# gkv856/speaker_embedding_GE2E_loss

Measured on NVIDIA B200. Metric: GE2E fwd+bwd utterances/s, higher is better.
Workload: dtype tf32

## Files before the change

### speaker_embedding_ge2e_loss_b200/csrc/ge2e_simt.cu

```cuda
#include <cuda_fp16.h>
#include <limits.h>

#include <algorithm>
#include <stdlib.h>

#include <initializer_list>

#include "ge2e_common.cuh"
#include "ge2e_tc_ptx.cuh"

namespace ge2e {

namespace {

constexpr int kThreads = 256;
constexpr int kWarps = kThreads / kWarp;
constexpr int kStreamRows = 32;

enum { MODE_FWD = 0, MODE_BWD_DE = 1, MODE_BWD_DC = 2 };

__device__ __forceinline__ float4 ld4(const float* __restrict__ row, int col, int D, bool vec) {
  float4 v = make_float4(0.f, 0.f, 0.f, 0.f);
  if (vec) {
    if (col < D) v = __ldg(reinterpret_cast<const float4*>(row + col));
// ... 67 lines not shown
  }
  __syncthreads();

  const float m1 = (float)(M - 1);
  for (int i = wid; i < M; i += kWarps) {
    float ne2 = 0.f, nu2 = 0.f, eu = 0.f;
    for (int d = lane << 2; d < Dp; d += 128) {
      const float4 e = *reinterpret_cast<const float4*>(&sE[(size_t)i * Dp + d]);
      const float4 s = *reinterpret_cast<const float4*>(&sS[d]);
      float4 u;
      u.x = (s.x - e.x) / m1; u.y = (s.y - e.y) / m1; u.z = (s.z - e.z) / m1; u.w = (s.w - e.w) / m1;
      ne2 += dot4(e, e);
      nu2 += dot4(u, u);
      eu += dot4(e, u);
    }
    ne2 = warp_sum(ne2); nu2 = warp_sum(nu2); eu = warp_sum(eu);
    const float inv_ne = 1.f / fmaxf(sqrtf(ne2), kCosDelta);
    const float inv_nu = 1.f / fmaxf(sqrtf(nu2), kCosDelta);
    float* out = e_hat + ((size_t)j * M + i) * D;
    for (int d = lane << 2; d < Dp; d += 128) {
      float4 e = *reinterpret_cast<const float4*>(&sE[(size_t)i * Dp + d]);
      e.x *= inv_ne; e.y *= inv_ne; e.z *= inv_ne; e.w *= inv_ne;
      if (ROUND) { e.x = round_tf32(e.x); e.y = round_tf32(e.y); e.z = round_tf32(e.z); e.w = round_tf32(e.w); }
      st4(out, d, D, vec_out, e);
    }
    if (lane == 0) cos_diag[(size_t)j * M + i] = eu * inv_ne * inv_nu;
  }

  float part = 0.f;
  const float fm = (float)M;
  for (int d = tid; d < Dp; d += kThreads) {
    const float c = sS[d] / fm;
    part += c * c;
  }
  const float tot = block_sum(part, red);
  if (tid == 0) s_inv_nc = 1.f / fmaxf(sqrtf(tot), kCosDelta);
  __syncthreads();
  const float inv_nc = s_inv_nc;
  for (int d = tid; d < D; d += kThreads) {
    float c = (sS[d] / fm) * inv_nc;
    if (ROUND) c = round_tf32(c);
    c_hat[(size_t)j * D + d] = c;
  }
}

template <bool ROUND>
__global__ void __launch_bounds__(kThreads)
prep_kernel(const float* __restrict__ E, const int32_t* __restrict__ idx, int M, int D, int Dp,
            float* __restrict__ e_hat, float* __restrict__ c_hat, float* __restrict__ cos_diag,
            float* __restrict__ accum) {
  extern __shared__ __align__(16) float smem[];
  if (blockIdx.x == 0 && threadIdx.x < 4 && accum != nullptr) accum[threadIdx.x] = 0.f;
  prep_body<ROUND>(E, idx, blockIdx.x, M, D, Dp, e_hat, c_hat, cos_diag, smem);
}


template <int PREC>
__device__ __forceinline__ void put4(float* base, size_t row, int D, int col, float4 v) {
  if (PREC == 3) {
    __half* h = reinterpret_cast<__half*>(base);
    const __half2 h0 = __floats2half2_rn(v.x, v.y), h1 = __floats2half2_rn(v.z, v.w);
    uint2 hi;
    hi.x = *reinterpret_cast<const uint32_t*>(&h0); hi.y = *reinterpret_cast<const uint32_t*>(&h1);
    *reinterpret_cast<uint2*>(h + row * 2 * D + col) = hi;
  } else if (PREC == 2) {
    __half* h = reinterpret_cast<__half*>(base);
    const __half2 h0 = __floats2half2_rn(v.x, v.y), h1 = __floats2half2_rn(v.z, v.w);
    const float2 f0 = __half22float2(h0), f1 = __half22float2(h1);
    const __half2 l0 = __floats2half2_rn(v.x - f0.x, v.y - f0.y), l1 = __floats2half2_rn(v.z - f1.x, v.w - f1.y);
    uint2 hi, lo;
    hi.x = *reinterpret_cast<const uint32_t*>(&h0); hi.y = *reinterpret_cast<const uint32_t*>(&h1);
    lo.x = *reinterpret_cast<const uint32_t*>(&l0); lo.y = *reinterpret_cast<const uint32_t*>(&l1);
    *reinterpret_cast<uint2*>(h + row * 2 * D + col) = hi;
    *reinterpret_cast<uint2*>(h + row * 2 * D + D + col) = lo;
  } else {
    if (PREC == 1) { v.x = round_tf32(v.x); v.y = round_tf32(v.y); v.z = round_tf32(v.z); v.w = round_tf32(v.w); }
    *reinterpret_cast<float4*>(base + row * D + col) = v;
  }
}

constexpr int kPrepWarps = 4;
constexpr int kRowBatch = 4;
constexpr int kRegRows = 16;

template <int KCH, int PREC>
__global__ void __launch_bounds__(kPrepWarps * 32)
prep_warp_kernel(const float* __restrict__ E, const int32_t* __restrict__ idx, int n_local, int M,
                 float* __restrict__ e_hat, float* __restrict__ c_hat, float* __restrict__ cos_diag,
                 float* __restrict__ accum) {
  constexpr int D = KCH * 128;
  const int lane = threadIdx.x & 31, wid = threadIdx.x >> 5;
  const int j = blockIdx.x * kPrepWarps + wid;
  pdl_wait();
  pdl_trigger();
  if (blockIdx.x == 0 && threadIdx.x < 4 && accum != nullptr) accum[threadIdx.x] = 0.f;
  if (j >= n_local) return;
  auto rowp = [&](int i) {
    return reinterpret_cast<const float4*>(E + phys_row(idx, (size_t)j * M + i) * D) + lane;
  };
  float4 s[KCH];
#pragma unroll
  for (int c = 0; c < KCH; ++c) s[c] = make_float4(0.f, 0.f, 0.f, 0.f);
  for (int i0 = 0; i0 < M; i0 += kRowBatch) {
    float4 v[kRowBatch][KCH];
#pragma unroll
    for (int r = 0; r < kRowBatch; ++r)
#pragma unroll
      for (int c = 0; c < KCH; ++c)
        v[r][c] = (i0 + r < M) ? __ldg(rowp(i0 + r) + c * 32) : make_float4(0.f, 0.f, 0.f, 0.f);
#pragma unroll
    for (int r = 0; r < kRowBatch; ++r)
#pragma unroll
      for (int c = 0; c < KCH; ++c) {
        s[c].x += v[r][c].x; s[c].y += v[r][c].y; s[c].z += v[r][c].z; s[c].w += v[r][c].w;
      }
  }
  const float inv_m = 1.f / (float)M, inv_m1 = 1.f / (float)(M - 1);
  float ss = 0.f;
#pragma unroll
  for (int c = 0; c < KCH; ++c) ss += dot4(s[c], s[c]);
  ss = warp_sum(ss);
  const float sc = inv_m / fmaxf(sqrtf(ss) * inv_m, kCosDelta);
#pragma unroll
  for (int c = 0; c < KCH; ++c)
    put4<PREC>(c_hat, j, D, 4 * lane + 128 * c,
               make_float4(s[c].x * sc, s[c].y * sc, s[c].z * sc, s[c].w * sc));
  float my_cos = 0.f;
  for (int i0 = 0; i0 < M; i0 += kRowBatch) {
    float4 v[kRowBatch][KCH];
    float ne2[kRowBatch], nd2[kRowBatch], ed[kRowBatch];
#pragma unroll
    for (int r = 0; r < kRowBatch; ++r)
#pragma unroll
      for (int c = 0; c < KCH; ++c)
        v[r][c] = (i0 + r < M) ? __ldg(rowp(i0 + r) + c * 32) : make_float4(0.f, 0.f, 0.f, 0.f);
#pragma unroll
    for (int r = 0; r < kRowBatch; ++r) {
      ne2[r] = 0.f; nd2[r] = 0.f; ed[r] = 0.f;
#pragma unroll
      for (int c = 0; c < KCH; ++c) {
        const float4 e = v[r][c];
        const float4 d = make_float4(s[c].x - e.x, s[c].y - e.y, s[c].z - e.z, s[c].w - e.w);
        ne2[r] += dot4(e, e); nd2[r] += dot4(d, d); ed[r] += dot4(e, d);
      }
    }
#pragma unroll
    for (int o = 16; o > 0; o >>= 1)
#pragma unroll
      for (int r = 0; r < kRowBatch; ++r) {
        ne2[r] += __shfl_xor_sync(0xffffffffu, ne2[r], o);
        nd2[r] += __shfl_xor_sync(0xffffffffu, nd2[r], o);
        ed[r] += __shfl_xor_sync(0xffffffffu, ed[r], o);
      }
#pragma unroll
    for (int r = 0; r < kRowBatch; ++r) {
      if (i0 + r < M) {
        const float inv_ne = 1.f / fmaxf(sqrtf(ne2[r]), kCosDelta);
        const float inv_nu = 1.f / fmaxf(sqrtf(nd2[r]) * inv_m1, kCosDelta);
        if (lane == ((i0 + r) & 31)) my_cos = (ed[r] * inv_m1) * inv_ne * inv_nu;
#pragma unroll
        for (int c = 0; c < KCH; ++c) {
          float4 e = v[r][c];
          e.x *= inv_ne; e.y *= inv_ne; e.z *= inv_ne; e.w *= inv_ne;
          put4<PREC>(e_hat, (size_t)j * M + i0 + r, D, 4 * lane + 128 * c, e);
        }
      }
    }
    if (((i0 + kRowBatch) & 31) == 0 || i0 + kRowBatch >= M) {
      const int base = (i0 + kRowBatch - 1) & ~31;
      if (base + lane < M) cos_diag[(size_t)j * M + base + lane] = my_cos;
    }
  }
}

__host__ __device__ constexpr int rev4(int i) {
  return ((i & 1) << 3) | ((i & 2) << 1) | ((i & 4) >> 1) | ((i & 8) >> 3);
}
__device__ __forceinline__ float reduce16_transposed(const float (&v)[16], int lane) {
  float a[8], b[4], c[2];
  const bool u1 = (lane & 1) != 0, u2 = (lane & 2) != 0, u4 = (lane & 4) != 0, u8 = (lane & 8) != 0;
#pragma unroll
  for (int q = 0; q < 8; ++q) a[q] = (u1 ? v[q + 8] : v[q]) + __shfl_xor_sync(0xffffffffu, u1 ? v[q] : v[q + 8], 1);
#pragma unroll
  for (int q = 0; q < 4; ++q) b[q] = (u2 ? a[q + 4] : a[q]) + __shfl_xor_sync(0xffffffffu, u2 ? a[q] : a[q + 4], 2);
#pragma unroll
  for (int q = 0; q < 2; ++q) c[q] = (u4 ? b[q + 2] : b[q]) + __shfl_xor_sync(0xffffffffu, u4 ? b[q] : b[q + 2], 4);
  const float e = (u8 ? c[1] : c[0]) + __shfl_xor_sync(0xffffffffu, u8 ? c[0] : c[1], 8);
  return e + __shfl_xor_sync(0xffffffffu, e, 16);
}

template <int KCH, int RR, int PREC>
__global__ void __launch_bounds__(kPrepWarps * 32)
prep_reg_kernel(const float* __restrict__ E, const int32_t* __restrict__ idx, int n_local, int M,
                float* __restrict__ e_hat, float* __restrict__ c_hat, float* __restrict__ cos_diag,
                float* __restrict__ accum) {
  constexpr int D = KCH * 128, R = RR;
  static_assert(R <= 16, "reduce16_transposed handles 16 rows");
  const int lane = threadIdx.x & 31, wid = threadIdx.x >> 5;
  const int j = blockIdx.x * kPrepWarps + wid;
  pdl_wait();
  pdl_trigger();
  if (blockIdx.x == 0 && threadIdx.x < 4 && accum != nullptr) accum[threadIdx.x] = 0.f;
  if (j >= n_local) return;
  float4 v[R][KCH];
#pragma unroll
  for (int i = 0; i < R; ++i) {
    const float4* rp = (i < M) ? reinterpret_cast<const float4*>(E + phys_row(idx, (size_t)j * M + i) * D) + lane : nullptr;
#pragma unroll
    for (int c = 0; c < KCH; ++c) v[i][c] = (i < M) ? __ldg(rp + c * 32) : make_float4(0.f, 0.f, 0.f, 0.f);
  }
  float4 s[KCH];
#pragma unroll
  for (int c = 0; c < KCH; ++c) {
    s[c] = v[0][c];
#pragma unroll
    for (int i = 1; i < R; ++i) { s[c].x += v[i][c].x; s[c].y += v[i][c].y; s[c].z += v[i][c].z; s[c].w += v[i][c].w; }
  }
  const float inv_m = 1.f / (float)M, inv_m1 = 1.f / (float)(M - 1);
  float ss = 0.f;
#pragma unroll
  for (int c = 0; c < KCH; ++c) ss += dot4(s[c], s[c]);
  ss = warp_sum(ss);
  const float sc = inv_m / fmaxf(sqrtf(ss) * inv_m, kCosDelta);
#pragma unroll
  for (int c = 0; c < KCH; ++c)
    put4<PREC>(c_hat, j, D, 4 * lane + 128 * c,
               make_float4(s[c].x * sc, s[c].y * sc, s[c].z * sc, s[c].w * sc));
  float ne2[16], nd2[16], ed[16];
#pragma unroll
  for (int i = R; i < 16; ++i) { ne2[i] = 0.f; nd2[i] = 0.f; ed[i] = 0.f; }
#pragma unroll
  for (int i = 0; i < R; ++i) {
    ne2[i] = 0.f; nd2[i] = 0.f; ed[i] = 0.f;
#pragma unroll
    for (int c = 0; c < KCH; ++c) {
      const float4 e = v[i][c];
      const float4 d = make_float4(s[c].x - e.x, s[c].y - e.y, s[c].z - e.z, s[c].w - e.w);
      ne2[i] += dot4(e, e); nd2[i] += dot4(d, d); ed[i] += dot4(e, d);
    }
  }
  const float t_ne2 = reduce16_transposed(ne2, lane), t_nd2 = reduce16_transposed(nd2, lane);
  const float t_ed = reduce16_transposed(ed, lane);
  const int my_row = rev4(lane & 15);
  const float inv_ne = 1.f / fmaxf(sqrtf(t_ne2), kCosDelta);
  const float inv_nu = 1.f / fmaxf(sqrtf(t_nd2) * inv_m1, kCosDelta);
  if (lane < 16 && my_row < M) cos_diag[(size_t)j * M + my_row] = (t_ed * inv_m1) * inv_ne * inv_nu;
#pragma unroll
  for (int i = 0; i < R; ++i) {
    if (i < M) {
      const float k = __shfl_sync(0xffffffffu, inv_ne, rev4(i));
#pragma unroll
      for (int c = 0; c < KCH; ++c) {
        float4 e = v[i][c];
        e.x *= k; e.y *= k; e.z *= k; e.w *= k;
        put4<PREC>(e_hat, (size_t)j * M + i, D, 4 * lane + 128 * c, e);
      }
    }
  }
}

struct StripParams {
  const float* own;
  const float* str;
  int n_own, n_str, D;
  int M, spk_offset;
  const float* cos_diag;
  const float* row_stat;
  const float* row_aux;
  float* row_aux_out;
  const float* w;
  const float* b;
  const float* grad_out;
  float eps;
  float* row_stat_out;
  int32_t* kstar_out;
  float* loss_accum;
  float* per_row_out;
  float* sim_out;
  float* acc_out;
  float* dwdb;
  int chunks_per_split;
};

template <int K, int R, int KCH>
struct RedT {
  static __device__ __forceinline__ void run(const float4 (&a)[R][KCH], const float* __restrict__ stage,
                                             int t, int lane, float (&out)[R]) {
    float lo[R], hi[R];
    RedT<K + 1, R, KCH>::run(a, stage, t, lane, lo);
    RedT<K + 1, R, KCH>::run(a, stage, t + (1 << K), lane, hi);
    const bool up = (lane & (1 << K)) != 0;
#pragma unroll
    for (int q = 0; q < R; ++q) {
      const float send = up ? lo[q] : hi[q];
      const float keep = up ? hi[q] : lo[q];
      out[q] = keep + __shfl_xor_sync(0xffffffffu, send, 1 << K);
    }
  }
};
template <int R, int KCH>
struct RedT<5, R, KCH> {
  static __device__ __forceinline__ void run(const float4 (&a)[R][KCH], const float* __restrict__ stage,
                                             int t, int lane, float (&out)[R]) {
#pragma unroll
    for (int q = 0; q < R; ++q) out[q] = 0.f;
#pragma unroll
    for (int c = 0; c < KCH; ++c) {
      const float4 bv = *reinterpret_cast<const float4*>(&stage[(size_t)t * (KCH * 128) + c * 128 + (lane << 2)]);
#pragma unroll
      for (int q = 0; q < R; ++q) out[q] += dot4(a[q][c], bv);
    }
  }
};

template <int MODE, int VARIANT, int KCH, int R>
__global__ void __launch_bounds__(kThreads)
strip_kernel(const StripParams p) {
  extern __shared__ __align__(16) float stage[];
  __shared__ float red[kWarps];
  constexpr int ROWLEN = KCH * 128;
  const int tid = threadIdx.x, lane = tid & 31, wid = tid >> 5;
  const int own0 = (blockIdx.x * kWarps + wid) * R;
  const int D = p.D;
  const bool vec_own = is_vec(p.own, D), vec_str = is_vec(p.str, D);
  const float w = __ldg(p.w), b = __ldg(p.b), eps = p.eps;
  const float g = (MODE == MODE_FWD) ? 1.f : __ldg(p.grad_out);

  float4 a[R][KCH];
#pragma unroll
  for (int q = 0; q < R; ++q) {
    const int row = own0 + q;
#pragma unroll
    for (int c = 0; c < KCH; ++c) {
      const int col = (lane << 2) + c * 128;
      a[q][c] = (row < p.n_own) ? ld4(p.own + (size_t)row * D, col, D, vec_own) : make_float4(0.f, 0.f, 0.f, 0.f);
    }
  }

  int jg[R];
// ... 420 lines not shown
    float ne2[kRowBatch], nd2[kRowBatch], ed[kRowBatch], eg[kRowBatch];
#pragma unroll
    for (int r = 0; r < kRowBatch; ++r) {
      ne2[r] = 0.f; nd2[r] = 0.f; ed[r] = 0.f; eg[r] = 0.f;
#pragma unroll
      for (int c = 0; c < KCH; ++c) {
        const bool in = i0 + r < M;
        v[r][c] = in ? __ldg(rowp(i0 + r) + c * 32) : make_float4(0.f, 0.f, 0.f, 0.f);
        const float4 gv = in ? __ldg(Gj + (size_t)(i0 + r) * (D / 4) + c * 32) : make_float4(0.f, 0.f, 0.f, 0.f);
        const float4 e = v[r][c];
        const float4 d = make_float4(s[c].x - e.x, s[c].y - e.y, s[c].z - e.z, s[c].w - e.w);
        ne2[r] += dot4(e, e); nd2[r] += dot4(d, d); ed[r] += dot4(e, d); eg[r] += dot4(e, gv);
      }
    }
#pragma unroll
    for (int o = 16; o > 0; o >>= 1)
#pragma unroll
      for (int r = 0; r < kRowBatch; ++r) {
        ne2[r] += __shfl_xor_sync(0xffffffffu, ne2[r], o);
        nd2[r] += __shfl_xor_sync(0xffffffffu, nd2[r], o);
        ed[r] += __shfl_xor_sync(0xffffffffu, ed[r], o);
        eg[r] += __shfl_xor_sync(0xffffffffu, eg[r], o);
      }
#pragma unroll
    for (int r = 0; r < kRowBatch; ++r) {
      if (i0 + r < M) {
        const int row = j * M + i0 + r;
        const float ne = sqrtf(ne2[r]), nu = sqrtf(nd2[r]) * inv_m1;
        const float inv_ne = 1.f / fmaxf(ne, kCosDelta), inv_nu = 1.f / fmaxf(nu, kCosDelta);
        const float cdv = (ed[r] * inv_m1) * inv_ne * inv_nu;
        float Gd;
        if (variant == GE2E_SOFTMAX) {
          Gd = -g * __ldg(row_aux + row);
        } else {
          const float sp = 1.f / (1.f + expf(-fmaf(w, __ldg(cos_diag + row) + eps, b)));
          Gd = -g * sp * (1.f - sp);
        }
        const float dd = w * Gd;
        const float gsc = row_scale != nullptr ? g * __ldcg(row_scale + row) : 1.f;
        float proj_e = eg[r] * gsc * inv_ne + dd * cdv;
        float proj_u = dd * cdv;
        if (ne < kCosDelta) proj_e *= clamp_proj_scale(ne);
        if (nu < kCosDelta) proj_u *= clamp_proj_scale(nu);
        const float r_ag = inv_ne * gsc;
        const float r_ad = dd * inv_nu * inv_m1 * inv_ne;
        const float r_ae = -proj_e * inv_ne * inv_ne;
        const float r_be = dd * inv_ne * inv_nu;
        const float r_bd = -proj_u * inv_nu * inv_nu * inv_m1;
        if (lane == i0 + r) { a_g = r_ag; a_e = r_ae; a_d = r_ad; b_e = r_be; b_d = r_bd; }
#pragma unroll
        for (int c = 0; c < KCH; ++c) {
          const float4 e = v[r][c];
          sd[c].x += r_be * e.x + r_bd * (s[c].x - e.x); sd[c].y += r_be * e.y + r_bd * (s[c].y - e.y);
          sd[c].z += r_be * e.z + r_bd * (s[c].z - e.z); sd[c].w += r_be * e.w + r_bd * (s[c].w - e.w);
        }
      }
    }
  }
  for (int i = 0; i < M; ++i) {
    float4* Oi = reinterpret_cast<float4*>(dE + phys_row(idx, (size_t)j * M + i) * D) + lane;
    const float r_ag = __shfl_sync(0xffffffffu, a_g, i), r_ae = __shfl_sync(0xffffffffu, a_e, i);
    const float r_ad = __shfl_sync(0xffffffffu, a_d, i), r_be = __shfl_sync(0xffffffffu, b_e, i);
    const float r_bd = __shfl_sync(0xffffffffu, b_d, i);
#pragma unroll
    for (int c = 0; c < KCH; ++c) {
      const float4 e = __ldg(rowp(i) + c * 32);
      const float4 gv = __ldg(Gj + (size_t)i * (D / 4) + c * 32);
      const float ev[4] = {e.x, e.y, e.z, e.w}, gg[4] = {gv.x, gv.y, gv.z, gv.w};
      const float sv[4] = {s[c].x, s[c].y, s[c].z, s[c].w}, sdv[4] = {sd[c].x, sd[c].y, sd[c].z, sd[c].w};
      const float bv[4] = {bc[c].x, bc[c].y, bc[c].z, bc[c].w};
      float o[4];
#pragma unroll
      for (int t = 0; t < 4; ++t) {
        const float d = sv[t] - ev[t];
        const float de = r_ag * gg[t] + r_ae * ev[t] + r_ad * d;
        const float du = r_be * ev[t] + r_bd * d;
        o[t] = de + bv[t] + (sdv[t] - du) * inv_m1;
      }
      Oi[c * 32] = make_float4(o[0], o[1], o[2], o[3]);
    }
  }
}

template <int KCH, int RR>
__global__ void __launch_bounds__(kPrepWarps * 32)
finalize_reg_kernel(const float* __restrict__ E, const float* __restrict__ dE_hat,
                    const float* __restrict__ dC_hat, const float* __restrict__ cos_diag,
                    const float* __restrict__ row_aux, const float* __restrict__ row_scale, int n_local, int M,
                    const float* __restrict__ wp, const float* __restrict__ bp, float eps, int variant,
                    const float* __restrict__ gp, float* __restrict__ dE, const int32_t* __restrict__ idx) {
  constexpr int D = KCH * 128, R = RR;
  static_assert(R <= 16, "reduce16_transposed handles 16 rows");
  const int lane = threadIdx.x & 31, wid = threadIdx.x >> 5;
  const int j = blockIdx.x * kPrepWarps + wid;
  const bool active = j < n_local;
  float4 v[R][KCH];
#pragma unroll
  for (int i = 0; i < R; ++i) {
    const bool in = active && i < M;
    const float4* rp = in ? reinterpret_cast<const float4*>(E + phys_row(idx, (size_t)j * M + i) * D) + lane : nullptr;
#pragma unroll
    for (int c = 0; c < KCH; ++c) v[i][c] = in ? __ldg(rp + c * 32) : make_float4(0.f, 0.f, 0.f, 0.f);
  }
  pdl_wait();
  pdl_trigger();
  if (!active) return;
  const float w = __ldg(wp), b = __ldg(bp), g = __ldg(gp);
  const float4* Gj = reinterpret_cast<const float4*>(dE_hat + (size_t)j * M * D) + lane;
  float4 s[KCH];
#pragma unroll
  for (int c = 0; c < KCH; ++c) {
    s[c] = v[0][c];
#pragma unroll
    for (int i = 1; i < R; ++i) { s[c].x += v[i][c].x; s[c].y += v[i][c].y; s[c].z += v[i][c].z; s[c].w += v[i][c].w; }
  }
  float t_ne2, t_nd2, t_ed, t_eg;
  {
    float q[16];
#pragma unroll
    for (int i = R; i < 16; ++i) q[i] = 0.f;
#pragma unroll
    for (int i = 0; i < R; ++i) {
      if (i == R / 2) asm volatile("" ::: "memory");
      q[i] = 0.f;
#pragma unroll
      for (int c = 0; c < KCH; ++c) {
        const float4 gv = (i < M) ? __ldg(Gj + (size_t)i * (D / 4) + c * 32) : make_float4(0.f, 0.f, 0.f, 0.f);
        q[i] += dot4(v[i][c], gv);
      }
    }
    t_eg = reduce16_transposed(q, lane);
#pragma unroll
    for (int i = 0; i < R; ++i) {
      q[i] = 0.f;
#pragma unroll
      for (int c = 0; c < KCH; ++c) q[i] += dot4(v[i][c], v[i][c]);
    }
    t_ne2 = reduce16_transposed(q, lane);
#pragma unroll
    for (int i = 0; i < R; ++i) {
      q[i] = 0.f;
#pragma unroll
      for (int c = 0; c < KCH; ++c) {
        const float4 e = v[i][c];
        const float4 d = make_float4(s[c].x - e.x, s[c].y - e.y, s[c].z - e.z, s[c].w - e.w);
        q[i] += dot4(d, d);
      }
    }
    t_nd2 = reduce16_transposed(q, lane);
#pragma unroll
    for (int i = 0; i < R; ++i) {
      q[i] = 0.f;
#pragma unroll
      for (int c = 0; c < KCH; ++c) {
        const float4 e = v[i][c];
        const float4 d = make_float4(s[c].x - e.x, s[c].y - e.y, s[c].z - e.z, s[c].w - e.w);
        q[i] += dot4(e, d);
      }
    }
    t_ed = reduce16_transposed(q, lane);
  }
  const float inv_m = 1.f / (float)M, inv_m1 = 1.f / (float)(M - 1);
  float4 bc[KCH];
  {
    float4 dch[KCH];
    float ss = 0.f, pr = 0.f;
#pragma unroll
    for (int c = 0; c < KCH; ++c) {
      dch[c] = __ldcg(reinterpret_cast<const float4*>(dC_hat + (size_t)j * D) + lane + c * 32);
      ss += dot4(s[c], s[c]);
      pr += dot4(s[c], dch[c]);
    }
    ss = warp_sum(ss); pr = warp_sum(pr);
    const float nc = sqrtf(ss) * inv_m;
    const float inv = 1.f / fmaxf(nc, kCosDelta);
    float proj = (pr * inv_m) * inv;
    if (nc < kCosDelta) proj *= clamp_proj_scale(nc);
    const float k1 = inv * inv_m;
    const float k2 = proj * inv * inv * inv_m * inv_m;
#pragma unroll
    for (int c = 0; c < KCH; ++c) {
      bc[c].x = dch[c].x * k1 - s[c].x * k2; bc[c].y = dch[c].y * k1 - s[c].y * k2;
      bc[c].z = dch[c].z * k1 - s[c].z * k2; bc[c].w = dch[c].w * k1 - s[c].w * k2;
    }
  }
  const int my_row = rev4(lane & 15);
  float a_g, a_e, a_d, b_e, b_d;
  {
    const int row = j * M + min(my_row, M - 1);
    const float ne = sqrtf(t_ne2), nu = sqrtf(t_nd2) * inv_m1;
    const float inv_ne = 1.f / fmaxf(ne, kCosDelta), inv_nu = 1.f / fmaxf(nu, kCosDelta);
    const float cdv = (t_ed * inv_m1) * inv_ne * inv_nu;
    float Gd;
    if (variant == GE2E_SOFTMAX) {
      Gd = -g * __ldcg(row_aux + row);
    } else {
      const float sp = 1.f / (1.f + expf(-fmaf(w, __ldg(cos_diag + row) + eps, b)));
      Gd = -g * sp * (1.f - sp);
    }
    const float dd = w * Gd;
    const float gsc = row_scale != nullptr ? g * __ldcg(row_scale + row) : 1.f;
    const float proj_e = t_eg * gsc * inv_ne + dd * cdv;
    const float proj_u = dd * cdv;
    a_g = inv_ne * gsc;
    a_d = dd * inv_nu * inv_m1 * inv_ne;
    a_e = -proj_e * inv_ne * inv_ne;
    b_e = dd * inv_ne * inv_nu;
    b_d = -proj_u * inv_nu * inv_nu * inv_m1;
    if (__any_sync(0xffffffffu, my_row < M && (ne < kCosDelta || nu < kCosDelta))) {
      a_e *= clamp_proj_scale(ne);
      b_d *= clamp_proj_scale(nu);
    }
  }
  float4 sd[KCH];
#pragma unroll
  for (int c = 0; c < KCH; ++c) sd[c] = make_float4(0.f, 0.f, 0.f, 0.f);
#pragma unroll
  for (int i = 0; i < R; ++i) {
    if (i < M) {
      const float r_be = __shfl_sync(0xffffffffu, b_e, rev4(i)), r_bd = __shfl_sync(0xffffffffu, b_d, rev4(i));
#pragma unroll
      for (int c = 0; c < KCH; ++c) {
        const float4 e = v[i][c];
        sd[c].x += r_be * e.x + r_bd * (s[c].x - e.x); sd[c].y += r_be * e.y + r_bd * (s[c].y - e.y);
        sd[c].z += r_be * e.z + r_bd * (s[c].z - e.z); sd[c].w += r_be * e.w + r_bd * (s[c].w - e.w);
      }
    }
  }
#pragma unroll
  for (int i = 0; i < R; ++i) {
    if (i < M) {
      float4* Oi = reinterpret_cast<float4*>(dE + phys_row(idx, (size_t)j * M + i) * D) + lane;
      const float r_ag = __shfl_sync(0xffffffffu, a_g, rev4(i)), r_ae = __shfl_sync(0xffffffffu, a_e, rev4(i));
      const float r_ad = __shfl_sync(0xffffffffu, a_d, rev4(i)), r_be = __shfl_sync(0xffffffffu, b_e, rev4(i));
      const float r_bd = __shfl_sync(0xffffffffu, b_d, rev4(i));
#pragma unroll
      for (int c = 0; c < KCH; ++c) {
        const float4 e = v[i][c];
        const float4 gv = __ldg(Gj + (size_t)i * (D / 4) + c * 32);
        const float ev[4] = {e.x, e.y, e.z, e.w}, gg[4] = {gv.x, gv.y, gv.z, gv.w};
        const float sv[4] = {s[c].x, s[c].y, s[c].z, s[c].w}, sdv[4] = {sd[c].x, sd[c].y, sd[c].z, sd[c].w};
        const float bv[4] = {bc[c].x, bc[c].y, bc[c].z, bc[c].w};
        float o[4];
#pragma unroll
        for (int t = 0; t < 4; ++t) {
          const float d = sv[t] - ev[t];
          const float de = r_ag * gg[t] + r_ae * ev[t] + r_ad * d;
          const float du = r_be * ev[t] + r_bd * d;
          o[t] = de + bv[t] + (sdv[t] - du) * inv_m1;
        }
        Oi[c * 32] = make_float4(o[0], o[1], o[2], o[3]);
      }
    }
  }
}

__global__ void centroids_kernel(const float* __restrict__ E, int M, int D, float* __restrict__ C) {
  const int j = blockIdx.x;
  for (int d = threadIdx.x; d < D; d += blockDim.x) {
    float s = 0.f;
    for (int i = 0; i < M; ++i) s += __ldg(E + ((size_t)j * M + i) * D + d);
    C[(size_t)j * D + d] = s / (float)M;
  }
}

__global__ void utt_centroids_kernel(const float* __restrict__ E, int M, int D, float* __restrict__ Uc) {
  const int j = blockIdx.x;
  const float m1 = (float)(M - 1);
  for (int d = threadIdx.x; d < D; d += blockDim.x) {
    float s = 0.f;
    for (int i = 0; i < M; ++i) s += __ldg(E + ((size_t)j * M + i) * D + d);
    for (int i = 0; i < M; ++i) {
      const size_t o = ((size_t)j * M + i) * D + d;
      Uc[o] = (s - __ldg(E + o)) / m1;
    }
  }
}

__global__ void normalize_rows_kernel(const float* __restrict__ X, int rows, int D, float* __restrict__ Y) {
  const int lane = threadIdx.x & 31, wid = threadIdx.x >> 5;
  const int r = blockIdx.x * (blockDim.x >> 5) + wid;
  if (r >= rows) return;
  float n2 = 0.f;
  for (int d = lane; d < D; d += 32) { const float v = __ldg(X + (size_t)r * D + d); n2 = fmaf(v, v, n2); }
  n2 = warp_sum(n2);
  const float inv = 1.f / fmaxf(sqrtf(n2), kCosDelta);
  for (int d = lane; d < D; d += 32) Y[(size_t)r * D + d] = __ldg(X + (size_t)r * D + d) * inv;
}

__global__ void __launch_bounds__(kThreads)
calc_loss_kernel(const float* __restrict__ S, int N, int M, float eps, int variant,
                 float* __restrict__ loss, float* __restrict__ per_row) {
  __shared__ float red[kWarps];
  const int tid = threadIdx.x, lane = tid & 31, wid = tid >> 5;
  const int r = blockIdx.x * kWarps + wid;
  float per = 0.f;
  if (r < N * M) {
    const int j = r / M;
    const float* row = S + (size_t)r * N;
    const float Sd = __ldg(row + j);
    if (variant == GE2E_SOFTMAX) {
      float mx = -INFINITY;
      for (int k = lane; k < N; k += 32) mx = fmaxf(mx, __ldg(row + k));
      mx = warp_max(mx);
      float l = 0.f;
      for (int k = lane; k < N; k += 32) l += expf(__ldg(row + k) - mx);
      l = warp_sum(l);
      const float lse = (mx > -80.f) ? mx + logf(l + eps * expf(-mx)) : logf(eps + l * expf(mx));
      per = lse - Sd;
    } else {
      float mx = -INFINITY;
      for (int k = lane; k < N; k += 32) if (k != j) mx = fmaxf(mx, __ldg(row + k));
      mx = warp_max(mx);
      per = 1.f - 1.f / (1.f + expf(-Sd));
      if (N > 1) per += 1.f / (1.f + expf(-mx));
    }
    if (lane == 0 && per_row != nullptr) per_row[r] = per;
    if (lane != 0) per = 0.f;
  }
  const float tot = block_sum(per, red);
  if (tid == 0) atomicAdd(loss, tot);
}

template <typename K>
int set_smem(K kernel, size_t bytes) {
  if (bytes > 48 * 1024)
    GE2E_CUDA_TRY(cudaFuncSetAttribute(kernel, cudaFuncAttributeMaxDynamicSharedMemorySize, (int)bytes));
  return GE2E_OK;
}

template <int MODE, int VARIANT, int KCH, int R>
int launch_strip(const StripParams& p, int splits, cudaStream_t st) {
  const size_t smem = (size_t)kStreamRows * KCH * 128 * sizeof(float);
  auto kern = strip_kernel<MODE, VARIANT, KCH, R>;
  int rc = set_smem(kern, smem);
  if (rc != GE2E_OK) return rc;
  dim3 grid((p.n_own + kWarps * R - 1) / (kWarps * R), splits);
  kern<<<grid, kThreads, smem, st>>>(p);
  GE2E_LAUNCHED();
  return GE2E_OK;
}

template <int MODE, int VARIANT>
int dispatch_strip(const StripParams& p, int splits, cudaStream_t st) {
  const int D = p.D;
  if (D <= 128) return launch_strip<MODE, VARIANT, 1, 4>(p, splits, st);
  if (D <= 256) return launch_strip<MODE, VARIANT, 2, 4>(p, splits, st);
  if (D <= 512) return launch_strip<MODE, VARIANT, 4, 2>(p, splits, st);
  if (D <= 1024) return launch_strip<MODE, VARIANT, 8, 1>(p, splits, st);
  return GE2E_ERR_UNSUPPORTED;
}

int rows_per_cta(int D) { return kWarps * (D <= 256 ? 4 : (D <= 512 ? 2 : 1)); }

}

constexpr size_t kGenericSmemCap = 200 * 1024;

int finalize_max_rows(int D) {
  if (D < 1 || D > 1024) return 0;
  const size_t row = (size_t)((D + 3) & ~3) * sizeof(float);
  return (int)(kGenericSmemCap / row / 2) - 1;
}

bool warp_path_ok(int D, std::initializer_list<const void*> ptrs) {
  if (D != 128 && D != 256 && D != 512) return false;
  for (const void* q : ptrs)
    if ((reinterpret_cast<uintptr_t>(q) & 15) != 0) return false;
  return true;
}

template <int KCH>
void launch_prep_warp(const float* E, const int32_t* idx, int n_local, int M, int prec, float* e_hat, float* c_hat,
                      float* cos_diag, float* accum, cudaStream_t st) {
  const int grid = (n_local + kPrepWarps - 1) / kPrepWarps;
  if (KCH <= 2 && M <= kRegRows) {
    constexpr int K2 = KCH <= 2 ? KCH : 1;
    const dim3 g(grid), bl(kPrepWarps * 32);
#define GE2E_PREP_REG(RR)                                                                                          \
  (prec == 3 ? launch_pdl(prep_reg_kernel<K2, RR, 3>, g, bl, 0, st, true, E, idx, n_local, M, e_hat, c_hat, cos_diag, accum) \
   : prec == 2 ? launch_pdl(prep_reg_kernel<K2, RR, 2>, g, bl, 0, st, true, E, idx, n_local, M, e_hat, c_hat, cos_diag, accum) \
   : prec == 1 ? launch_pdl(prep_reg_kernel<K2, RR, 1>, g, bl, 0, st, true, E, idx, n_local, M, e_hat, c_hat, cos_diag, accum) \
               : launch_pdl(prep_reg_kernel<K2, RR, 0>, g, bl, 0, st, true, E, idx, n_local, M, e_hat, c_hat, cos_diag, accum))
    if (M <= 4) GE2E_PREP_REG(4); else if (M <= 8) GE2E_PREP_REG(8); else if (M <= 12) GE2E_PREP_REG(12); else GE2E_PREP_REG(16);
#undef GE2E_PREP_REG
    return;
  }
  if (prec == 3) launch_pdl(prep_warp_kernel<KCH, 3>, dim3(grid), dim3(kPrepWarps * 32), 0, st, true, E, idx, n_local, M,
                            e_hat, c_hat, cos_diag, accum);
  else if (prec == 2) launch_pdl(prep_warp_kernel<KCH, 2>, dim3(grid), dim3(kPrepWarps * 32), 0, st, true, E, idx, n_local, M,
                            e_hat, c_hat, cos_diag, accum);
  else if (prec == 1) launch_pdl(prep_warp_kernel<KCH, 1>, dim3(grid), dim3(kPrepWarps * 32), 0, st, true, E, idx, n_local,
                                 M, e_hat, c_hat, cos_diag, accum);
  else launch_pdl(prep_warp_kernel<KCH, 0>, dim3(grid), dim3(kPrepWarps * 32), 0, st, true, E, idx, n_local, M,
                  e_hat, c_hat, cos_diag, accum);
}

template <int KCH>
void launch_finalize_warp(const float* E, const float* dE_hat, const float* dC_hat, const float* cos_diag,
                          const float* row_aux, const float* row_scale, int n_local, int M, const float* w,
                          const float* b, float eps,
                          int variant, const float* g, float* dE, const int32_t* idx, bool pdl, cudaStream_t st) {
  const int grid = (n_local + kPrepWarps - 1) / kPrepWarps;
  if (KCH <= 2 && M <= kRegRows) {
    constexpr int K2 = KCH <= 2 ? KCH : 1;
#define GE2E_FIN_REG(RR)                                                                                     \
  launch_pdl(finalize_reg_kernel<K2, RR>, dim3(grid), dim3(kPrepWarps * 32), 0, st, pdl, E, dE_hat, dC_hat, cos_diag, \
             row_aux, row_scale, n_local, M, w, b, eps, variant, g, dE, idx)
    if (M <= 4) GE2E_FIN_REG(4); else if (M <= 8) GE2E_FIN_REG(8); else if (M <= 12) GE2E_FIN_REG(12); else GE2E_FIN_REG(16);
#undef GE2E_FIN_REG
    return;
  }
  launch_pdl(finalize_warp_kernel<KCH>, dim3(grid), dim3(kPrepWarps * 32), 0, st, pdl, E, dE_hat, dC_hat, cos_diag,
             row_aux, row_scale, n_local, M, w, b, eps, variant, g, dE, idx);
}

int simt_prep(const float* E, const int32_t* row_index, int n_local, int M, int D, int prec, float* e_hat,
              float* c_hat_local, float* cos_diag, float* accum, cudaStream_t st) {
  const bool round_tf32_ = prec == 1;
  if (warp_path_ok(D, {E, e_hat, c_hat_local})) {
    if (D == 128) launch_prep_warp<1>(E, row_index, n_local, M, prec, e_hat, c_hat_local, cos_diag, accum, st);
    else if (D == 256) launch_prep_warp<2>(E, row_index, n_local, M, prec, e_hat, c_hat_local, cos_diag, accum, st);
    else launch_prep_warp<4>(E, row_index, n_local, M, prec, e_hat, c_hat_local, cos_diag, accum, st);
    GE2E_LAUNCHED();
    return GE2E_OK;
  }
  if (prec >= 2) return GE2E_ERR_UNSUPPORTED;
  const int Dp = (D + 3) & ~3;
  const size_t smem = (size_t)(M + 1) * Dp * sizeof(float);
  if (smem > kGenericSmemCap) return GE2E_ERR_UNSUPPORTED;
  if (round_tf32_) {
    int rc = set_smem(prep_kernel<true>, smem);
    if (rc != GE2E_OK) return rc;
    prep_kernel<true><<<n_local, kThreads, smem, st>>>(E, row_index, M, D, Dp, e_hat, c_hat_local, cos_diag, accum);
  } else {
    int rc = set_smem(prep_kernel<false>, smem);
    if (rc != GE2E_OK) return rc;
    prep_kernel<false><<<n_local, kThreads, smem, st>>>(E, row_index, M, D, Dp, e_hat, c_hat_local, cos_diag, accum);
  }
  GE2E_LAUNCHED();
  return GE2E_OK;
}

int simt_fwd_rows(const RowsArgs& a, float* row_stat, int32_t* row_kstar, float* row_aux, float* loss_accum,
                  float* per_row_out, float* sim_out, cudaStream_t st) {
  StripParams p{};
  p.own = a.e_hat; p.n_own = a.n_local * a.M;
  p.str = a.c_hat_all; p.n_str = a.n_total;
  p.D = a.D; p.M = a.M; p.spk_offset = a.spk_offset;
  p.cos_diag = a.cos_diag; p.w = a.w; p.b = a.b; p.eps = a.eps;
  p.row_stat_out = row_stat; p.kstar_out = row_kstar; p.row_aux_out = row_aux; p.loss_accum = loss_accum;
  p.per_row_out = per_row_out; p.sim_out = sim_out;
  p.chunks_per_split = INT_MAX / 2;
  if (a.variant == GE2E_SOFTMAX) return dispatch_strip<MODE_FWD, GE2E_SOFTMAX>(p, 1, st);
  return dispatch_strip<MODE_FWD, GE2E_CONTRAST>(p, 1, st);
}

int simt_bwd_rows(const RowsArgs& a, const float* row_stat, const int32_t* row_kstar, const float* row_aux,
                  const float* grad_out, float* dE_hat, float* dC_hat_partial, float* dwdb_accum,
                  cudaStream_t st) {
  const int U = a.n_local * a.M;
  const size_t dc_elems = (size_t)a.n_total * a.D;
  if (dwdb_accum == dC_hat_partial + dc_elems) {
    GE2E_CUDA_TRY(cudaMemsetAsync(dC_hat_partial, 0, (dc_elems + 2) * sizeof(float), st));
  } else {
    GE2E_CUDA_TRY(cudaMemsetAsync(dC_hat_partial, 0, dc_elems * sizeof(float), st));
    GE2E_CUDA_TRY(cudaMemsetAsync(dwdb_accum, 0, 2 * sizeof(float), st));
  }
  if (a.variant == GE2E_CONTRAST) {
    contrast_bwd_kernel<<<(U + kWarps - 1) / kWarps, kThreads, 0, st>>>(
        a.e_hat, a.c_hat_all, a.cos_diag, row_stat, row_kstar, U, a.D, a.w, a.b, a.eps, grad_out,
        dE_hat, dC_hat_partial, dwdb_accum);
    GE2E_LAUNCHED();
    return GE2E_OK;
  }
  StripParams p{};
  p.D = a.D; p.M = a.M; p.spk_offset = a.spk_offset;
  p.cos_diag = a.cos_diag; p.row_stat = row_stat; p.row_aux = row_aux; p.w = a.w; p.b = a.b; p.grad_out = grad_out;
  p.eps = a.eps;
  p.own = a.e_hat; p.n_own = U; p.str = a.c_hat_all; p.n_str = a.n_total;
  p.acc_out = dE_hat; p.dwdb = dwdb_accum; p.chunks_per_split = INT_MAX / 2;
  int rc = dispatch_strip<MODE_BWD_DE, GE2E_SOFTMAX>(p, 1, st);
  if (rc != GE2E_OK) return rc;
  p.own = a.c_hat_all; p.n_own = a.n_total; p.str = a.e_hat; p.n_str = U;
  p.acc_out = dC_hat_partial; p.dwdb = nullptr;
  const int own_ctas = (a.n_total + rows_per_cta(a.D) - 1) / rows_per_cta(a.D);
  const int nchunks = (U + kStreamRows - 1) / kStreamRows;
  int splits = (2 * 148 + own_ctas - 1) / own_ctas;
  splits = max(1, min(splits, nchunks));
  p.chunks_per_split = (nchunks + splits - 1) / splits;
  splits = (nchunks + p.chunks_per_split - 1) / p.chunks_per_split;
// ... 1000 lines not shown
```

Before: 152.7 million.

## Split each speaker across W warps in prep/finalize register kernels

The register-resident prep and finalize kernels now assign one warp per 128-column slice of a speaker, so D=256 uses two warps per speaker. Partial reductions are combined through shared memory with a named barrier per speaker group. This halves per-thread register arrays, and launch bounds now request four blocks per SM to raise occupancy. Finalize also hoists the PDL-independent statistics ahead of pdl_wait and folds the output arithmetic into fewer coefficients, at the cost of an extra barrier and shared-memory exchange.

```diff
diff --git a/speaker_embedding_ge2e_loss_b200/csrc/ge2e_simt.cu b/speaker_embedding_ge2e_loss_b200/csrc/ge2e_simt.cu
--- a/speaker_embedding_ge2e_loss_b200/csrc/ge2e_simt.cu
+++ b/speaker_embedding_ge2e_loss_b200/csrc/ge2e_simt.cu
@@ -173,6 +173,7 @@
 constexpr int kPrepWarps = 4;
 constexpr int kRowBatch = 4;
 constexpr int kRegRows = 16;
+constexpr int kRegBlocksPerSM = 4;
 
 template <int KCH, int PREC>
 __global__ void __launch_bounds__(kPrepWarps * 32)
@@ -280,72 +281,75 @@
   return e + __shfl_xor_sync(0xffffffffu, e, 16);
 }
 
-template <int KCH, int RR, int PREC>
-__global__ void __launch_bounds__(kPrepWarps * 32)
+template <int W, int Q>
+__device__ __forceinline__ void speaker_sum(float (&x)[Q], float (*xch)[Q][16], int wid, int lane) {
+  if (W == 1) return;
+  if (lane < 16) {
+#pragma unroll
+    for (int q = 0; q < Q; ++q) xch[wid][q][lane] = x[q];
+  }
+  asm volatile("bar.sync %0, %1;" ::"r"(1 + wid / W), "r"(W * 32) : "memory");
+  const int first = wid - wid % W;
+#pragma unroll
+  for (int q = 0; q < Q; ++q) {
+    float t = xch[first][q][lane & 15];
+#pragma unroll
+    for (int w = 1; w < W; ++w) t += xch[first + w][q][lane & 15];
+    x[q] = t;
+  }
+}
+
+template <int W, int RR, int PREC>
+__global__ void __launch_bounds__(kPrepWarps * 32, kRegBlocksPerSM)
 prep_reg_kernel(const float* __restrict__ E, const int32_t* __restrict__ idx, int n_local, int M,
                 float* __restrict__ e_hat, float* __restrict__ c_hat, float* __restrict__ cos_diag,
                 float* __restrict__ accum) {
-  constexpr int D = KCH * 128, R = RR;
+  constexpr int D = W * 128, R = RR;
   static_assert(R <= 16, "reduce16_transposed handles 16 rows");
+  static_assert(kPrepWarps % W == 0, "a block holds whole speakers");
+  __shared__ float xch[kPrepWarps][4][16];
   const int lane = threadIdx.x & 31, wid = threadIdx.x >> 5;
-  const int j = blockIdx.x * kPrepWarps + wid;
+  const int j = blockIdx.x * (kPrepWarps / W) + wid / W;
+  const int col = 128 * (wid % W) + 4 * lane;
   pdl_wait();
   pdl_trigger();
   if (blockIdx.x == 0 && threadIdx.x < 4 && accum != nullptr) accum[threadIdx.x] = 0.f;
   if (j >= n_local) return;
-  float4 v[R][KCH];
+  float4 v[R];
+#pragma unroll
+  for (int i = 0; i < R; ++i)
+    v[i] = (i < M) ? __ldg(reinterpret_cast<const float4*>(E + phys_row(idx, (size_t)j * M + i) * D + col))
+                   : make_float4(0.f, 0.f, 0.f, 0.f);
+  float4 s = v[0];
+#pragma unroll
+  for (int i = 1; i < R; ++i) { s.x += v[i].x; s.y += v[i].y; s.z += v[i].z; s.w += v[i].w; }
+  const float inv_m = 1.f / (float)M, inv_m1 = 1.f / (float)(M - 1);
+  float ne2[16], nd2[16], ed[16];
+#pragma unroll
+  for (int i = R; i < 16; ++i) { ne2[i] = 0.f; nd2[i] = 0.f; ed[i] = 0.f; }
 #pragma unroll
   for (int i = 0; i < R; ++i) {
-    const float4* rp = (i < M) ? reinterpret_cast<const float4*>(E + phys_row(idx, (size_t)j * M + i) * D) + lane : nullptr;
-#pragma unroll
-    for (int c = 0; c < KCH; ++c) v[i][c] = (i < M) ? __ldg(rp + c * 32) : make_float4(0.f, 0.f, 0.f, 0.f);
-  }
-  float4 s[KCH];
-#pragma unroll
-  for (int c = 0; c < KCH; ++c) {
-    s[c] = v[0][c];
-#pragma unroll
-    for (int i = 1; i < R; ++i) { s[c].x += v[i][c].x; s[c].y += v[i][c].y; s[c].z += v[i][c].z; s[c].w += v[i][c].w; }
-  }
-  const float inv_m = 1.f / (float)M, inv_m1 = 1.f / (float)(M - 1);
-  float ss = 0.f;
-#pragma unroll
-  for (int c = 0; c < KCH; ++c) ss += dot4(s[c], s[c]);
-  ss = warp_sum(ss);
-  const float sc = inv_m / fmaxf(sqrtf(ss) * inv_m, kCosDelta);
-#pragma unroll
-  for (int c = 0; c < KCH; ++c)
-    put4<PREC>(c_hat, j, D, 4 * lane + 128 * c,
-               make_float4(s[c].x * sc, s[c].y * sc, s[c].z * sc, s[c].w * sc));
-  float ne2[16], nd2[16], ed[16];
-#pragma unroll
-  for (int i = R; i < 16; ++i) { ne2[i] = 0.f; nd2[i] = 0.f; ed[i] = 0.f; }
-#pragma unroll
-  for (int i = 0; i < R; ++i) {
-    ne2[i] = 0.f; nd2[i] = 0.f; ed[i] = 0.f;
-#pragma unroll
-    for (int c = 0; c < KCH; ++c) {
-      const float4 e = v[i][c];
-      const float4 d = make_float4(s[c].x - e.x, s[c].y - e.y, s[c].z - e.z, s[c].w - e.w);
-      ne2[i] += dot4(e, e); nd2[i] += dot4(d, d); ed[i] += dot4(e, d);
-    }
-  }
-  const float t_ne2 = reduce16_transposed(ne2, lane), t_nd2 = reduce16_transposed(nd2, lane);
-  const float t_ed = reduce16_transposed(ed, lane);
+    const float4 e = v[i];
+    const float4 d = make_float4(s.x - e.x, s.y - e.y, s.z - e.z, s.w - e.w);
+    ne2[i] = dot4(e, e); nd2[i] = dot4(d, d); ed[i] = dot4(e, d);
+  }
+  float t[4] = {reduce16_transposed(ne2, lane), reduce16_transposed(nd2, lane), reduce16_transposed(ed, lane),
+                warp_sum(dot4(s, s))};
+  speaker_sum<W>(t, xch, wid, lane);
+  const float sc = inv_m / fmaxf(sqrtf(t[3]) * inv_m, kCosDelta);
+  put4<PREC>(c_hat, j, D, col, make_float4(s.x * sc, s.y * sc, s.z * sc, s.w * sc));
   const int my_row = rev4(lane & 15);
-  const float inv_ne = 1.f / fmaxf(sqrtf(t_ne2), kCosDelta);
-  const float inv_nu = 1.f / fmaxf(sqrtf(t_nd2) * inv_m1, kCosDelta);
-  if (lane < 16 && my_row < M) cos_diag[(size_t)j * M + my_row] = (t_ed * inv_m1) * inv_ne * inv_nu;
+  const float inv_ne = 1.f / fmaxf(sqrtf(t[0]), kCosDelta);
+  const float inv_nu = 1.f / fmaxf(sqrtf(t[1]) * inv_m1, kCosDelta);
+  if (wid % W == 0 && lane < 16 && my_row < M)
+    cos_diag[(size_t)j * M + my_row] = (t[2] * inv_m1) * inv_ne * inv_nu;
 #pragma unroll
   for (int i = 0; i < R; ++i) {
     if (i < M) {
       const float k = __shfl_sync(0xffffffffu, inv_ne, rev4(i));
-#pragma unroll
-      for (int c = 0; c < KCH; ++c) {
-        float4 e = v[i][c];
-        e.x *= k; e.y *= k; e.z *= k; e.w *= k;
-        put4<PREC>(e_hat, (size_t)j * M + i, D, 4 * lane + 128 * c, e);
-      }
+      float4 e = v[i];
+      e.x *= k; e.y *= k; e.z *= k; e.w *= k;
+      put4<PREC>(e_hat, (size_t)j * M + i, D, col, e);
     }
   }
 }
@@ -932,124 +936,89 @@
   }
 }
 
-template <int KCH, int RR>
-__global__ void __launch_bounds__(kPrepWarps * 32)
+template <int W, int RR>
+__global__ void __launch_bounds__(kPrepWarps * 32, kRegBlocksPerSM)
 finalize_reg_kernel(const float* __restrict__ E, const float* __restrict__ dE_hat,
                     const float* __restrict__ dC_hat, const float* __restrict__ cos_diag,
                     const float* __restrict__ row_aux, const float* __restrict__ row_scale, int n_local, int M,
                     const float* __restrict__ wp, const float* __restrict__ bp, float eps, int variant,
                     const float* __restrict__ gp, float* __restrict__ dE, const int32_t* __restrict__ idx) {
-  constexpr int D = KCH * 128, R = RR;
+  constexpr int D = W * 128, R = RR;
   static_assert(R <= 16, "reduce16_transposed handles 16 rows");
+  static_assert(kPrepWarps % W == 0, "a block holds whole speakers");
+  __shared__ float xch[kPrepWarps][6][16];
   const int lane = threadIdx.x & 31, wid = threadIdx.x >> 5;
-  const int j = blockIdx.x * kPrepWarps + wid;
+  const int j = blockIdx.x * (kPrepWarps / W) + wid / W;
+  const int col = 128 * (wid % W) + 4 * lane;
   const bool active = j < n_local;
-  float4 v[R][KCH];
-#pragma unroll
-  for (int i = 0; i < R; ++i) {
-    const bool in = active && i < M;
-    const float4* rp = in ? reinterpret_cast<const float4*>(E + phys_row(idx, (size_t)j * M + i) * D) + lane : nullptr;
-#pragma unroll
-    for (int c = 0; c < KCH; ++c) v[i][c] = in ? __ldg(rp + c * 32) : make_float4(0.f, 0.f, 0.f, 0.f);
+  float4 v[R];
+#pragma unroll
+  for (int i = 0; i < R; ++i)
+    v[i] = (active && i < M) ? __ldg(reinterpret_cast<const float4*>(E + phys_row(idx, (size_t)j * M + i) * D + col))
+                             : make_float4(0.f, 0.f, 0.f, 0.f);
+  float4 s = v[0];
+#pragma unroll
+  for (int i = 1; i < R; ++i) { s.x += v[i].x; s.y += v[i].y; s.z += v[i].z; s.w += v[i].w; }
+  float t[6];
+  {
+    float ne2[16], nd2[16], ed[16];
+#pragma unroll
+    for (int i = R; i < 16; ++i) { ne2[i] = 0.f; nd2[i] = 0.f; ed[i] = 0.f; }
+#pragma unroll
+    for (int i = 0; i < R; ++i) {
+      const float4 e = v[i];
+      const float4 d = make_float4(s.x - e.x, s.y - e.y, s.z - e.z, s.w - e.w);
+      ne2[i] = dot4(e, e); nd2[i] = dot4(d, d); ed[i] = dot4(e, d);
+    }
+    t[1] = reduce16_transposed(ne2, lane); t[2] = reduce16_transposed(nd2, lane); t[3] = reduce16_transposed(ed, lane);
+    t[4] = warp_sum(dot4(s, s));
   }
   pdl_wait();
   pdl_trigger();
   if (!active) return;
   const float w = __ldg(wp), b = __ldg(bp), g = __ldg(gp);
-  const float4* Gj = reinterpret_cast<const float4*>(dE_hat + (size_t)j * M * D) + lane;
-  float4 s[KCH];
-#pragma unroll
-  for (int c = 0; c < KCH; ++c) {
-    s[c] = v[0][c];
-#pragma unroll
-    for (int i = 1; i < R; ++i) { s[c].x += v[i][c].x; s[c].y += v[i][c].y; s[c].z += v[i][c].z; s[c].w += v[i][c].w; }
-  }
-  float t_ne2, t_nd2, t_ed, t_eg;
+  const int my_row = rev4(lane & 15);
+  const int row = j * M + min(my_row, M - 1);
+  const float4 dch = __ldcg(reinterpret_cast<const float4*>(dC_hat + (size_t)j * D + col));
+  const float aux = variant == GE2E_SOFTMAX ? __ldcg(row_aux + row) : __ldg(cos_diag + row);
+  const float gsc = row_scale != nullptr ? g * __ldcg(row_scale + row) : 1.f;
+  const float* Gj = dE_hat + (size_t)j * M * D + col;
   {
-    float q[16];
-#pragma unroll
-    for (int i = R; i < 16; ++i) q[i] = 0.f;
-#pragma unroll
-    for (int i = 0; i < R; ++i) {
-      if (i == R / 2) asm volatile("" ::: "memory");
-      q[i] = 0.f;
-#pragma unroll
-      for (int c = 0; c < KCH; ++c) {
-        const float4 gv = (i < M) ? __ldg(Gj + (size_t)i * (D / 4) + c * 32) : make_float4(0.f, 0.f, 0.f, 0.f);
-        q[i] += dot4(v[i][c], gv);
-      }
-    }
-    t_eg = reduce16_transposed(q, lane);
-#pragma unroll
-    for (int i = 0; i < R; ++i) {
-      q[i] = 0.f;
-#pragma unroll
-      for (int c = 0; c < KCH; ++c) q[i] += dot4(v[i][c], v[i][c]);
-    }
-    t_ne2 = reduce16_transposed(q, lane);
-#pragma unroll
-    for (int i = 0; i < R; ++i) {
-      q[i] = 0.f;
-#pragma unroll
-      for (int c = 0; c < KCH; ++c) {
-        const float4 e = v[i][c];
-        const float4 d = make_float4(s[c].x - e.x, s[c].y - e.y, s[c].z - e.z, s[c].w - e.w);
-        q[i] += dot4(d, d);
-      }
-    }
-    t_nd2 = reduce16_transposed(q, lane);
-#pragma unroll
-    for (int i = 0; i < R; ++i) {
-      q[i] = 0.f;
-#pragma unroll
-      for (int c = 0; c < KCH; ++c) {
-        const float4 e = v[i][c];
-        const float4 d = make_float4(s[c].x - e.x, s[c].y - e.y, s[c].z - e.z, s[c].w - e.w);
-        q[i] += dot4(e, d);
-      }
-    }
-    t_ed = reduce16_transposed(q, lane);
-  }
+    float eg[16];
+#pragma unroll
+    for (int i = R; i < 16; ++i) eg[i] = 0.f;
+#pragma unroll
+    for (int i = 0; i < R; ++i)
+      eg[i] = dot4(v[i], (i < M) ? __ldg(reinterpret_cast<const float4*>(Gj + (size_t)i * D)) : make_float4(0.f, 0.f, 0.f, 0.f));
+    t[0] = reduce16_transposed(eg, lane);
+    t[5] = warp_sum(dot4(s, dch));
+  }
+  speaker_sum<W>(t, xch, wid, lane);
+  const float t_eg = t[0], t_ne2 = t[1], t_nd2 = t[2], t_ed = t[3];
   const float inv_m = 1.f / (float)M, inv_m1 = 1.f / (float)(M - 1);
-  float4 bc[KCH];
+  float4 bc;
   {
-    float4 dch[KCH];
-    float ss = 0.f, pr = 0.f;
-#pragma unroll
-    for (int c = 0; c < KCH; ++c) {
-      dch[c] = __ldcg(reinterpret_cast<const float4*>(dC_hat + (size_t)j * D) + lane + c * 32);
-      ss += dot4(s[c], s[c]);
-      pr += dot4(s[c], dch[c]);
-    }
-    ss = warp_sum(ss); pr = warp_sum(pr);
-    const float nc = sqrtf(ss) * inv_m;
+    const float nc = sqrtf(t[4]) * inv_m;
     const float inv = 1.f / fmaxf(nc, kCosDelta);
-    float proj = (pr * inv_m) * inv;
+    float proj = (t[5] * inv_m) * inv;
     if (nc < kCosDelta) proj *= clamp_proj_scale(nc);
     const float k1 = inv * inv_m;
     const float k2 = proj * inv * inv * inv_m * inv_m;
-#pragma unroll
-    for (int c = 0; c < KCH; ++c) {
-      bc[c].x = dch[c].x * k1 - s[c].x * k2; bc[c].y = dch[c].y * k1 - s[c].y * k2;
-      bc[c].z = dch[c].z * k1 - s[c].z * k2; bc[c].w = dch[c].w * k1 - s[c].w * k2;
-    }
-  }
-  const int my_row = rev4(lane & 15);
+    bc = make_float4(dch.x * k1 - s.x * k2, dch.y * k1 - s.y * k2, dch.z * k1 - s.z * k2, dch.w * k1 - s.w * k2);
+  }
   float a_g, a_e, a_d, b_e, b_d;
   {
-    const int row = j * M + min(my_row, M - 1);
     const float ne = sqrtf(t_ne2), nu = sqrtf(t_nd2) * inv_m1;
     const float inv_ne = 1.f / fmaxf(ne, kCosDelta), inv_nu = 1.f / fmaxf(nu, kCosDelta);
     const float cdv = (t_ed * inv_m1) * inv_ne * inv_nu;
     float Gd;
     if (variant == GE2E_SOFTMAX) {
-      Gd = -g * __ldcg(row_aux + row);
+      Gd = -g * aux;
     } else {
-      const float sp = 1.f / (1.f + expf(-fmaf(w, __ldg(cos_diag + row) + eps, b)));
+      const float sp = 1.f / (1.f + expf(-fmaf(w, aux + eps, b)));
       Gd = -g * sp * (1.f - sp);
     }
     const float dd = w * Gd;
-    const float gsc = row_scale != nullptr ? g * __ldcg(row_scale + row) : 1.f;
     const float proj_e = t_eg * gsc * inv_ne + dd * cdv;
     const float proj_u = dd * cdv;
     a_g = inv_ne * gsc;
@@ -1062,45 +1031,30 @@
       b_d *= clamp_proj_scale(nu);
     }
   }
-  float4 sd[KCH];
-#pragma unroll
-  for (int c = 0; c < KCH; ++c) sd[c] = make_float4(0.f, 0.f, 0.f, 0.f);
+  float4 sd = make_float4(0.f, 0.f, 0.f, 0.f);
 #pragma unroll
   for (int i = 0; i < R; ++i) {
     if (i < M) {
       const float r_be = __shfl_sync(0xffffffffu, b_e, rev4(i)), r_bd = __shfl_sync(0xffffffffu, b_d, rev4(i));
-#pragma unroll
-      for (int c = 0; c < KCH; ++c) {
-        const float4 e = v[i][c];
-        sd[c].x += r_be * e.x + r_bd * (s[c].x - e.x); sd[c].y += r_be * e.y + r_bd * (s[c].y - e.y);
-        sd[c].z += r_be * e.z + r_bd * (s[c].z - e.z); sd[c].w += r_be * e.w + r_bd * (s[c].w - e.w);
-      }
-    }
-  }
+      const float4 e = v[i];
+      sd.x += r_be * e.x + r_bd * (s.x - e.x); sd.y += r_be * e.y + r_bd * (s.y - e.y);
+      sd.z += r_be * e.z + r_bd * (s.z - e.z); sd.w += r_be * e.w + r_bd * (s.w - e.w);
+    }
+  }
+  const float k_s = a_d - b_d * inv_m1;
+  const float k_e = a_e - b_e * inv_m1 - k_s;
+  const float4 base = make_float4(fmaf(sd.x, inv_m1, bc.x), fmaf(sd.y, inv_m1, bc.y), fmaf(sd.z, inv_m1, bc.z),
+                                  fmaf(sd.w, inv_m1, bc.w));
 #pragma unroll
   for (int i = 0; i < R; ++i) {
     if (i < M) {
-      float4* Oi = reinterpret_cast<float4*>(dE + phys_row(idx, (size_t)j * M + i) * D) + lane;
-      const float r_ag = __shfl_sync(0xffffffffu, a_g, rev4(i)), r_ae = __shfl_sync(0xffffffffu, a_e, rev4(i));
-      const float r_ad = __shfl_sync(0xffffffffu, a_d, rev4(i)), r_be = __shfl_sync(0xffffffffu, b_e, rev4(i));
-      const float r_bd = __shfl_sync(0xffffffffu, b_d, rev4(i));
-#pragma unroll
-      for (int c = 0; c < KCH; ++c) {
-        const float4 e = v[i][c];
-        const float4 gv = __ldg(Gj + (size_t)i * (D / 4) + c * 32);
-        const float ev[4] = {e.x, e.y, e.z, e.w}, gg[4] = {gv.x, gv.y, gv.z, gv.w};
-        const float sv[4] = {s[c].x, s[c].y, s[c].z, s[c].w}, sdv[4] = {sd[c].x, sd[c].y, sd[c].z, sd[c].w};
-        const float bv[4] = {bc[c].x, bc[c].y, bc[c].z, bc[c].w};
-        float o[4];
-#pragma unroll
-        for (int t = 0; t < 4; ++t) {
-          const float d = sv[t] - ev[t];
-          const float de = r_ag * gg[t] + r_ae * ev[t] + r_ad * d;
-          const float du = r_be * ev[t] + r_bd * d;
-          o[t] = de + bv[t] + (sdv[t] - du) * inv_m1;
-        }
-        Oi[c * 32] = make_float4(o[0], o[1], o[2], o[3]);
-      }
+      const float r_g = __shfl_sync(0xffffffffu, a_g, rev4(i)), r_e = __shfl_sync(0xffffffffu, k_e, rev4(i));
+      const float r_s = __shfl_sync(0xffffffffu, k_s, rev4(i));
+      const float4 e = v[i];
+      const float4 gv = __ldg(reinterpret_cast<const float4*>(Gj + (size_t)i * D));
+      const float4 o = make_float4(r_g * gv.x + r_e * e.x + fmaf(r_s, s.x, base.x), r_g * gv.y + r_e * e.y + fmaf(r_s, s.y, base.y),
+                                   r_g * gv.z + r_e * e.z + fmaf(r_s, s.z, base.z), r_g * gv.w + r_e * e.w + fmaf(r_s, s.w, base.w));
+      *reinterpret_cast<float4*>(dE + phys_row(idx, (size_t)j * M + i) * D + col) = o;
     }
   }
 }
@@ -1225,13 +1179,13 @@
                       float* cos_diag, float* accum, cudaStream_t st) {
   const int grid = (n_local + kPrepWarps - 1) / kPrepWarps;
   if (KCH <= 2 && M <= kRegRows) {
-    constexpr int K2 = KCH <= 2 ? KCH : 1;
-    const dim3 g(grid), bl(kPrepWarps * 32);
+    constexpr int W = KCH <= 2 ? KCH : 1, spb = kPrepWarps / W;
+    const dim3 g((n_local + spb - 1) / spb), bl(kPrepWarps * 32);
 #define GE2E_PREP_REG(RR)                                                                                          \
-  (prec == 3 ? launch_pdl(prep_reg_kernel<K2, RR, 3>, g, bl, 0, st, true, E, idx, n_local, M, e_hat, c_hat, cos_diag, accum) \
-   : prec == 2 ? launch_pdl(prep_reg_kernel<K2, RR, 2>, g, bl, 0, st, true, E, idx, n_local, M, e_hat, c_hat, cos_diag, accum) \
-   : prec == 1 ? launch_pdl(prep_reg_kernel<K2, RR, 1>, g, bl, 0, st, true, E, idx, n_local, M, e_hat, c_hat, cos_diag, accum) \
-               : launch_pdl(prep_reg_kernel<K2, RR, 0>, g, bl, 0, st, true, E, idx, n_local, M, e_hat, c_hat, cos_diag, accum))
+  (prec == 3 ? launch_pdl(prep_reg_kernel<W, RR, 3>, g, bl, 0, st, true, E, idx, n_local, M, e_hat, c_hat, cos_diag, accum) \
+   : prec == 2 ? launch_pdl(prep_reg_kernel<W, RR, 2>, g, bl, 0, st, true, E, idx, n_local, M, e_hat, c_hat, cos_diag, accum) \
+   : prec == 1 ? launch_pdl(prep_reg_kernel<W, RR, 1>, g, bl, 0, st, true, E, idx, n_local, M, e_hat, c_hat, cos_diag, accum) \
+               : launch_pdl(prep_reg_kernel<W, RR, 0>, g, bl, 0, st, true, E, idx, n_local, M, e_hat, c_hat, cos_diag, accum))
     if (M <= 4) GE2E_PREP_REG(4); else if (M <= 8) GE2E_PREP_REG(8); else if (M <= 12) GE2E_PREP_REG(12); else GE2E_PREP_REG(16);
 #undef GE2E_PREP_REG
     return;
@@ -1253,10 +1207,11 @@
                           int variant, const float* g, float* dE, const int32_t* idx, bool pdl, cudaStream_t st) {
   const int grid = (n_local + kPrepWarps - 1) / kPrepWarps;
   if (KCH <= 2 && M <= kRegRows) {
-    constexpr int K2 = KCH <= 2 ? KCH : 1;
+    constexpr int W = KCH <= 2 ? KCH : 1, spb = kPrepWarps / W;
+    const dim3 gr((n_local + spb - 1) / spb), bl(kPrepWarps * 32);
 #define GE2E_FIN_REG(RR)                                                                                     \
-  launch_pdl(finalize_reg_kernel<K2, RR>, dim3(grid), dim3(kPrepWarps * 32), 0, st, pdl, E, dE_hat, dC_hat, cos_diag, \
-             row_aux, row_scale, n_local, M, w, b, eps, variant, g, dE, idx)
+  launch_pdl(finalize_reg_kernel<W, RR>, gr, bl, 0, st, pdl, E, dE_hat, dC_hat, cos_diag, row_aux, row_scale, n_local, M, \
+             w, b, eps, variant, g, dE, idx)
     if (M <= 4) GE2E_FIN_REG(4); else if (M <= 8) GE2E_FIN_REG(8); else if (M <= 12) GE2E_FIN_REG(12); else GE2E_FIN_REG(16);
 #undef GE2E_FIN_REG
     return;
```

New measurement: 166.6 million, median of 6. +9.2%, better.
